# okieraised/rs-face-detection-tflite

Measured on AMD Instinct MI355X. Metric: faces/sec at batch=256 (256x256 back-camera) per GPU, higher is better.
Workload: dtype f32

## Files before the change

rs-face-detection-tflite_amd/csrc/engine.cpp:

```cpp
#include "engine.hpp"
#include "launch.hpp"

#include <algorithm>
#include <cstdio>
#include <cstdlib>
#include <cstring>
#include <stdexcept>

namespace mi {

void hip_check(hipError_t e, const char* what) {
    if (e != hipSuccess) throw std::runtime_error(std::string(what) + ": " + hipGetErrorString(e));
}

namespace {
template <class T>
void upload(T*& dev, std::vector<T>& host, const char* what_alloc, const char* what_copy) {
    if (dev) hip_check(hipFree(dev), "hipFree");
    dev = nullptr;
    if (host.empty()) return;
    hip_check(hipMalloc(reinterpret_cast<void**>(&dev), host.size() * sizeof(T)), what_alloc);
    hip_check(hipMemcpy(dev, host.data(), host.size() * sizeof(T), hipMemcpyHostToDevice), what_copy);
    std::vector<T>().swap(host);
}
// ... 53 lines not shown

const Model::Option* Model::find_option(const std::string& key) {
    using O = Option;
    constexpr int kMax = 0x7fffffff;
    static const Option table[] = {
        {"chunk", &Model::chunk_, 0, kMax, 0},
        {"graph", &Model::use_graph_, 0, 1, 0},
        {"fuse", &Model::fuse_level_, 0, 5, O::kReplan},
        {"res_budget", &Model::res_budget_, 16, 156, O::kReplan | O::kKiB},
        {"pipe", &Model::pipe_max_, 0, 4, O::kReplan},
        {"small_chain", &Model::small_chain_, 0, 64, O::kFreeSmall},
        {"pipe_rows", &Model::pipe_rows_, 1 << 1 | 1 << 2 | 1 << 4, 0, O::kOneOf},
        {"pipe_band", &Model::pipe_band_, 0, 4096, 0},
        {"strip", &Model::strip_, 0, 1, 0},
        {"stem_fuse", &Model::stem_fuse_, 0, 1, 0},
        {"stem_mfma", &Model::stem_mfma_, 0, 2, O::kForms},
        {"conv_mfma", &Model::conv_mfma_, 0, 1, 0},
        {"conv_bf16", &Model::conv_bf16_, 0, 2, O::kReplan},
        {"stem_run", &Model::stem_run_, 0, 32, 0},
        {"pair_fuse", &Model::pair_fuse_, 0, 1, 0},
        {"mdb_band", &Model::mdb_band_, 0, 4096, 0},
        {"chain_fixed", &Model::chain_fixed_, 0, 1, 0},
        {"chain_sched", &Model::chain_sched_, 0, 1, 0},
        {"mchain", &Model::mchain_, 0, 1, 0},
        {"tail", &Model::tail_, 0, 1, O::kReplan},
        {"tail_pre", &Model::tail_pre_, 0, 2, 0},
        {"tail_g", &Model::tail_g_, 0, 64, 0},
        {"band", &Model::band_, 0, 2, O::kReplan},
        {"band_test_fail", &Model::band_test_fail_, 0, 1, O::kWriteOnly},
        {"band_test_absent", &Model::band_test_absent_, 0, 256, O::kWriteOnly},
        {"band_test_gen", nullptr, 0, kMax, O::kBandGen | O::kWriteOnly},
        {"band_wide", &Model::band_wide_ok_, 0, 1, O::kReplan},
        {"band_fork", &Model::band_fork_, 0, 1, O::kReplan},
        {"band_nw", &Model::band_nw_, 8, 256, O::kReplan},
        {"band_fail_streak", &Model::band_fail_streak_, 0, 0, O::kReadOnly},
        {"band_wraps", &Model::band_wraps_, 0, 0, O::kReadOnly},
        {"fork", &Model::fork_, 0, 1, 0},
        {"heads", &Model::head_streams_opt_, 1, kHeadStreams, O::kReplan},
        {"reuse", &Model::reuse_, 0, 1, O::kReplan},
        {"lanes", &Model::lanes_, 1, 4, 0},
        {"test_poison", &Model::test_poison_, 1 << 1 | 1 << 2, 0, O::kOneOf | O::kKeepGraphs},
    };
    for (const Option& o : table)
        if (key == o.key) return &o;
    return nullptr;
}
// ... 198 lines not shown
}

LaunchCtx Model::launch_ctx(const float* in, int chunk_start, int frames) const {
    LaunchCtx c;
    c.weights = d_weights_;
    c.arena = d_arena_ + static_cast<size_t>(plan_.arena_floats_per_frame) * chunk_cap_ * arena_lane_;
    c.in = in; c.out = d_out_.data();
    c.small = d_small_; c.small_floats = small_floats_;
    c.progs = d_programs_; c.tail_progs = d_tail_programs_;
    c.band_prog = d_band_prog_; c.band_consts = d_band_consts_; c.band_ws = d_band_ws_; c.band_sync = d_band_sync_; c.band_fail = d_band_fail_;
    c.chunk_cap = chunk_cap_; c.chunk_start = chunk_start; c.F = frames;
    c.u8_frames = u8_.frames; c.u8_lut = u8_.lut; c.u8_frame_bytes = u8_.frame_bytes; c.u8_row_bytes = u8_.row_bytes;
    c.strip = strip_; c.pair_fuse = pair_fuse_; c.stem_fuse = stem_fuse_; c.stem_mfma = stem_mfma_; c.stem_run = stem_run_; c.mchain = mchain_; c.conv_mfma = conv_mfma_; c.conv_bf16 = conv_bf16_;
    c.small_chain = small_chain_; c.lanes = lanes_;
    c.pipe_rows = pipe_rows_; c.pipe_band = pipe_band_; c.mdb_band = mdb_band_; c.tail_pre = tail_pre_; c.tail_g = tail_g_;
    c.fork = fork_ && lanes_ == 1;
    c.cu_count = device_cu_count();
    c.band = band_use_ && chunk_start == 0;
    c.band_test_absent = band_test_absent_;
    return c;
}

namespace {
int issue(const Launch& l, hipStream_t s, int chain_fixed, int chain_sched) {
    auto many = [&](int (*f)(const BlockArgs*, int, void*)) { return f(l.blocks.data(), static_cast<int>(l.blocks.size()), s); };
    switch (l.to) {
        case Launcher::Conv: return launch_conv(std::get<ConvArgs>(l.args), s);
        case Launcher::HeadGemm: return launch_head_gemm(std::get<HeadGemmArgs>(l.args), s);
        case Launcher::Dw: return launch_dw(std::get<DwArgs>(l.args), s);
        case Launcher::Xc: return launch_xc(std::get<XcArgs>(l.args), s);
        case Launcher::Mdblock: return launch_mdblock(std::get<DblockArgs>(l.args), s);
        case Launcher::Dblock: return launch_dblock(std::get<DblockArgs>(l.args), s);
        case Launcher::Mbneck: return launch_mbneck(std::get<BneckArgs>(l.args), s);
        case Launcher::Bneck: return launch_bneck(std::get<BneckArgs>(l.args), s);
        case Launcher::Tail: return launch_tail(std::get<TailLaunch>(l.args), s);
        case Launcher::Resident: return launch_resident(std::get<ResLaunch>(l.args), s);
        case Launcher::Chain: return launch_chain(std::get<ChainArgs>(l.args), s, chain_fixed, chain_sched);
        case Launcher::StripPipe: return many(launch_strip_pipe);
        case Launcher::MstripChain: return many(launch_mstrip_chain);
        case Launcher::SmallChain: {
            int rc = 0;
            for (size_t k = 0; k < l.blocks.size() && rc == 0; k++) rc = l.blocks[k].sh == 1 ? launch_strip(l.blocks[k], s) : launch_block(l.blocks[k], s);
            return rc;
        }
        case Launcher::Ms2: return launch_ms2(std::get<BlockArgs>(l.args), s);
        case Launcher::Mwalk: return launch_mwalk(std::get<BlockArgs>(l.args), s);
        case Launcher::Strip: return launch_strip(std::get<BlockArgs>(l.args), s);
        case Launcher::Mstrip: return launch_mstrip(std::get<BlockArgs>(l.args), s);
        case Launcher::Block: return launch_block(std::get<BlockArgs>(l.args), s);
        case Launcher::Add: return launch_add(std::get<EltArgs>(l.args), s);
        case Launcher::Act: return launch_act(std::get<EltArgs>(l.args), s);
        case Launcher::Maxpool: return launch_maxpool(std::get<EltArgs>(l.args), s);
        case Launcher::Padc: return launch_padc(std::get<EltArgs>(l.args), s);
        case Launcher::Resize2x: return launch_resize2x(std::get<EltArgs>(l.args), s);
        case Launcher::DepthToSpace: return launch_depth_to_space(std::get<EltArgs>(l.args), s);
        case Launcher::Bandnet: return launch_bandnet(std::get<BandLaunch>(l.args), s);
        case Launcher::Avgpool: return launch_avgpool(std::get<EltArgs>(l.args), s);
        case Launcher::L2norm: return launch_l2norm_rows(std::get<EltArgs>(l.args), s);
        case Launcher::Transpose: return launch_transpose(std::get<EltArgs>(l.args), s);
    }
    return 0;
}
}

void Model::enqueue_chunk(const float* in, int chunk_start, int F, hipStream_t trunk, std::vector<hipEvent_t>* marks, Lowered* keep) {
    LaunchCtx ctx = launch_ctx(in, chunk_start, F);
    if (marks) ctx.fork = false;
    Lowered low = lower_chunk(plan_, consts_, band_plan_, sched_, ctx, keep != nullptr);
    auto mark = [&] {
        if (!marks) return;
        hipEvent_t ev;
// ... 8 lines not shown
        if (!head_events_[k]) hip_check(hipEventCreateWithFlags(&head_events_[k], hipEventDisableTiming), "hipEventCreate");
        return head_events_[k];
    };
    unsigned used_heads = 0;
    for (size_t k = 0; k < n_launches; k++) {
        const Launch& l = low.launches[k];
        hipStream_t s = trunk;
        if (l.slot >= 0) {
            while (static_cast<int>(head_streams_.size()) <= l.slot) {
                hipStream_t st;
                hip_check(hipStreamCreateWithFlags(&st, hipStreamNonBlocking), "hipStreamCreate");
                head_streams_.push_back(st);
            }
            s = head_streams_[static_cast<size_t>(l.slot)];
            if (l.wait >= 0) {
                hip_check(wait_event(s, event(static_cast<size_t>(low.launch_of_node[static_cast<size_t>(l.wait)]))), "hipStreamWaitEvent");
            } else {
                hip_check(record_event(event(start_event), trunk), "hipEventRecord");
                hip_check(wait_event(s, event(start_event)), "hipStreamWaitEvent");
            }
            used_heads |= 1u << l.slot;
        }
        int rc = 0;
        for (int rep = 0; rep < (marks ? profile_inner_ : 1) && rc == 0; rep++) rc = issue(l, s, chain_fixed_, chain_sched_);
        if (rc != 0) throw std::runtime_error(std::string("kernel launch failed: ") + hipGetErrorString(static_cast<hipError_t>(rc)));
        if (l.record) hip_check(record_event(event(k), s), "hipEventRecord");
        mark();
    }
    for (int k = 0; k < kHeadStreams; k++)
        if (used_heads & (1u << k)) {
            hip_check(record_event(event(start_event + 1 + static_cast<size_t>(k)), head_streams_[static_cast<size_t>(k)]), "hipEventRecord");
            hip_check(wait_event(trunk, event(start_event + 1 + static_cast<size_t>(k))), "hipStreamWaitEvent");
        }
    last_chunk_frames_ = F;
    if (keep) *keep = std::move(low);
}

void Model::enqueue_all(const float* in, int batch, hipStream_t s) {
    if (lanes_ > 1 && batch > chunk_cap_) {
        while (static_cast<int>(side_streams_.size()) < lanes_ - 1) {
            hipStream_t st;
            hip_check(hipStreamCreateWithFlags(&st, hipStreamNonBlocking), "hipStreamCreate");
            side_streams_.push_back(st);
        }
        while (static_cast<int>(lane_events_.size()) < lanes_) {
            hipEvent_t ev;
            hip_check(hipEventCreateWithFlags(&ev, hipEventDisableTiming), "hipEventCreate");
// ... 197 lines not shown
```

rs-face-detection-tflite_amd/csrc/engine.hpp:

```cpp
#pragma once

#include <hip/hip_runtime.h>

#include <map>
#include <memory>
#include <string>
#include <vector>

#include "bandplan.hpp"
#include "consts.hpp"
#include "launches.hpp"
#include "plan.hpp"

namespace mi {

void hip_check(hipError_t e, const char* what);

class Model {
   public:
    Model(const uint8_t* bytes, size_t n, int device);
    ~Model();
    Model(const Model&) = delete;
    Model& operator=(const Model&) = delete;

// ... 29 lines not shown
    void rebuild();
    struct Option;
    static const Option* find_option(const std::string& key);
    void build_bandnet();
    void free_bandnet();
    bool band_usable(int batch) const;
    void band_before_launch(hipStream_t s);
    void poison_scratch(hipStream_t s);
    void ensure_capacity(int batch);
    LaunchCtx launch_ctx(const float* in, int chunk_start, int frames) const;
    void enqueue_chunk(const float* in, int chunk_start, int frames, hipStream_t s, std::vector<hipEvent_t>* marks = nullptr, Lowered* keep = nullptr);
    void enqueue_all(const float* in, int batch, hipStream_t s);
    void invalidate_graphs();

    int device_ = 0;
    std::vector<uint8_t> blob_;
    Plan plan_;
    int fuse_level_ = 5, pipe_max_ = 4, tail_ = 1, reuse_ = 1;
    int res_budget_ = 156 * 1024;
    int chunk_ = 0, lanes_ = 1, use_graph_ = 1;
    int fork_ = 1, head_streams_opt_ = 1;
    int conv_mfma_ = 1;
    int conv_bf16_ = 0;
    int strip_ = 1, stem_fuse_ = 1, stem_mfma_ = 1, stem_run_ = 0, pair_fuse_ = 1, mchain_ = 1, chain_fixed_ = 1, chain_sched_ = 1;
    int pipe_rows_ = 0, pipe_band_ = 0, mdb_band_ = 0;
    int tail_pre_ = 0, tail_g_ = 0;
    int arena_lane_ = 0;
    std::vector<hipStream_t> side_streams_;
    std::vector<hipEvent_t> lane_events_;
    SideSchedule sched_;
    std::vector<hipStream_t> head_streams_;
    std::vector<hipEvent_t> head_events_;
    bool dirty_ = true;

    float* d_weights_ = nullptr;
    PlanConsts consts_;
    int profile_inner_ = 1;

    ResStage* d_programs_ = nullptr;
    TailStage* d_tail_programs_ = nullptr;
    float* d_arena_ = nullptr;
    size_t arena_floats_ = 0;
    int chunk_cap_ = 0;
    int batch_cap_ = 0;
    std::vector<float*> d_out_;
    float* d_in_stage_ = nullptr;
    size_t in_stage_floats_ = 0;
// ... 54 lines not shown
```

rs-face-detection-tflite_amd/csrc/kernels.hpp:

```cpp
#pragma once

#include <cstddef>
#include <cstdint>

namespace mi {

enum ActKind : int { ACT_NONE = 0, ACT_RELU = 1, ACT_RELU6 = 2, ACT_PRELU = 3 };
enum ResMode : int { RES_NONE = 0, RES_DIRECT = 1, RES_MAXPOOL = 2, RES_UP2X = 3 };

struct Epilogue {
    const float* bias = nullptr;
    const float* alpha = nullptr;
    const float* res = nullptr;
    long res_fs = 0;
    int res_mode = RES_NONE;
    int res_C = 0;
    int res_W = 0, res_H = 0;
    int act = ACT_NONE;
    int res_after = 0;
};

struct ConvArgs {
    const float* in = nullptr;
    const uint8_t* in_u8 = nullptr;
// ... 246 lines not shown
int launch_conv_bf16(const ConvArgs& a, void* stream);
int launch_dw(const DwArgs& a, void* stream);
int launch_block(const BlockArgs& a, void* stream);
bool block_kernel_supports(const BlockArgs& a);
const char* block_kernel_label(const BlockArgs& a, char* buf, size_t cap);
int launch_strip(const BlockArgs& a, void* stream);
bool strip_kernel_supports(const BlockArgs& a);
bool strip_shape_ok(int C, int Co);
int strip_consts_floats(int C);
void strip_pack_consts(int C, const float* w_dw, const float* b_dw, const float* w_pw, const float* bias, const float* alpha, int act, float* dst);
const char* strip_kernel_label(const BlockArgs& a, char* buf, size_t cap);
int launch_mwalk(const BlockArgs& a, void* stream);
bool mwalk_kernel_supports(const BlockArgs& a);
bool mwalk_shape_ok(int W, int C, int Co);
int mwalk_consts_floats(int W, int C, int Co);
void mwalk_pack_consts(int W, int C, int Co, const float* w_dw, const float* b_dw, const float* w_pw, const float* bias, const float* alpha, int act, float* dst);
const char* mwalk_kernel_label(const BlockArgs& a, char* buf, size_t cap);
int launch_ms2(const BlockArgs& a, void* stream);
bool ms2_kernel_supports(const BlockArgs& a);
bool ms2_shape_ok(int W, int C, int Co, bool skip);
int ms2_consts_floats(int W, int C, int Co, bool skip);
void ms2_pack_consts(int W, int C, int Co, bool skip, const float* w_dw, const float* b_dw, const float* w_pw, const float* bias, const float* alpha, int act, float* dst);
const char* ms2_kernel_label(const BlockArgs& a, char* buf, size_t cap);
int launch_mstrip(const BlockArgs& a, void* stream);
bool mstrip_kernel_supports(const BlockArgs& a);
bool mstrip_shape_ok(int C, int Co);
int mstrip_consts_floats(int C);
void mstrip_pack_consts(int C, const float* w_dw, const float* b_dw, const float* w_pw, const float* bias, const float* alpha, int act, float* dst);
const char* mstrip_kernel_label(const BlockArgs& a, char* buf, size_t cap);
bool mstrip_chain_supports(const BlockArgs* blocks, int n);
int launch_mstrip_chain(const BlockArgs* blocks, int n, void* stream);
bool strip_pipe_supports(const BlockArgs* blocks, int n);
bool strip_pipe_shape_ok(int C, int W);
bool strip_tail_shape_ok(int C, int Co, int H, int W);
int strip_consts_s2_floats(int C, int Co);
void strip_pack_consts_s2(int C, int Co, const float* w_dw, const float* b_dw, const float* w_pw, const float* bias, const float* alpha, int act, float* dst);
int launch_strip_pipe(const BlockArgs* blocks, int n, void* stream);
const char* strip_pipe_label(const BlockArgs* blocks, int n, char* buf, size_t cap);
int strip_pipe_rows_per_step(int H, int hint = 0);
int launch_chain(const ChainArgs& a, void* stream, int fixed = 1, int sched = 1);

struct BneckBlock {
    const float* w1 = nullptr;
    const float* w2 = nullptr;
    const float* consts = nullptr;
    float hi1 = 0.f, hi2 = 0.f;
    const float* mconsts = nullptr;
    int act1 = ACT_RELU, act2 = ACT_RELU;
};
constexpr int kMaxBneck = 6;
struct BneckArgs {
    const float* in = nullptr;
    float* out = nullptr;
    long in_fs = 0, out_fs = 0;
// ... 163 lines not shown
```

rs-face-detection-tflite_amd/csrc/mrow.hpp:

```cpp
#pragma once

#include <hip/hip_runtime.h>

#include <type_traits>
#include <utility>

#include "kernels.hpp"
#include "launch.hpp"
#include "wave_sync.hpp"

namespace mi {

namespace {

typedef float df32x4 __attribute__((ext_vector_type(4)));

__device__ __forceinline__ void dwg_barrier() {
    asm volatile("s_waitcnt lgkmcnt(0)\n\ts_barrier" ::: "memory");
}

template <class F, int... KS>
__device__ __forceinline__ void dfor_each(F&& f, std::integer_sequence<int, KS...>) { (f(std::integral_constant<int, KS>{}), ...); }

typedef float dv2f __attribute__((ext_vector_type(2)));
// ... 1 lines not shown
template <int WT>
struct RowAcc {
    dv2f p[WT / 2 ? WT / 2 : 1];
    float s[1];
    __device__ __forceinline__ void clear() {
#pragma unroll
        for (int q = 0; q < (WT / 2 ? WT / 2 : 1); q++) p[q] = dv2f{0.f, 0.f};
        s[0] = 0.f;
    }
};

template <int S>
__device__ __forceinline__ void dpk_fma(dv2f& acc, const dv2f x, const dv2f w) {
    if constexpr (S == 0) asm volatile("v_pk_fma_f32 %0, %1, %2, %0 op_sel:[0,0,0] op_sel_hi:[1,0,1]" : "+v"(acc) : "v"(x), "v"(w));
    else asm volatile("v_pk_fma_f32 %0, %1, %2, %0 op_sel:[0,1,0] op_sel_hi:[1,1,1]" : "+v"(acc) : "v"(x), "v"(w));
}
template <int S>
__device__ __forceinline__ dv2f dpk_mul(const dv2f x, const dv2f w) {
    dv2f r;
    if constexpr (S == 0) asm volatile("v_pk_mul_f32 %0, %1, %2 op_sel:[0,0] op_sel_hi:[1,0]" : "=v"(r) : "v"(x), "v"(w));
    else asm volatile("v_pk_mul_f32 %0, %1, %2 op_sel:[0,1] op_sel_hi:[1,1]" : "=v"(r) : "v"(x), "v"(w));
    return r;
}

__device__ __forceinline__ void dtaps_from(const float4 t0, const float4 t1, const float4 t2, dv2f (&t)[5]) {
    t[0] = dv2f{t0.x, t0.y}; t[1] = dv2f{t0.z, t0.w}; t[2] = dv2f{t1.x, t1.y}; t[3] = dv2f{t1.z, t1.w}; t[4] = dv2f{t2.x, 0.f};
}
template <int CK>
__device__ __forceinline__ void dload_taps(const float4* tp, dv2f (&tap)[CK][5]) {
#pragma unroll
    for (int ks = 0; ks < CK; ks++) dtaps_from(tp[ks * 12], tp[ks * 12 + 1], tp[ks * 12 + 2], tap[ks]);
#pragma unroll
    for (int ks = 0; ks < CK; ks++)
#pragma unroll
        for (int t = 0; t < 5; t++) asm volatile("" : "+v"(tap[ks][t]));
}

template <int CK, int MT, int WT, int PSV, bool EMIT, bool TAPL = false>
__device__ __forceinline__ void mdb_row(const unsigned src, const unsigned aop, const dv2f (&tap)[TAPL ? 1 : CK][5], RowAcc<WT> (&aPN)[CK], RowAcc<WT> (&aC)[CK],
                                        df32x4 (&D)[MT][WT], const float4* tapl = nullptr) {
    constexpr int NP = WT / 2, ODD = WT & 1;
    float xs[2][3][WT], av[2][MT];
    auto load_ks = [&](auto ksc, float (&x)[3][WT], float (&aw)[MT]) {
        constexpr int ks = decltype(ksc)::value;
        const unsigned xa = src, aa = aop;
#pragma unroll
// ... 89 lines not shown
        if constexpr (EMIT) {
#pragma unroll
            for (int mt = 0; mt < MT; mt++) asm volatile("ds_read_b32 %0, %1 offset:%2" : "=v"(aw[mt]) : "v"(aa), "n"((ks * MT + mt) * 64 * 4));
        }
    };
    auto landed = [&](float (&x)[3][2], float (&aw)[MT]) {
#pragma unroll
        for (int dx = 0; dx < 3; dx++) asm volatile("" : "+v"(x[dx][0]), "+v"(x[dx][1]));
        if constexpr (EMIT) {
#pragma unroll
            for (int mt = 0; mt < MT; mt++) asm volatile("" : "+v"(aw[mt]));
        }
    };
    auto kstep = [&](auto ksc) {
        constexpr int ks = decltype(ksc)::value;
        if constexpr (ks + 1 < CK) load_ks(std::integral_constant<int, ks + 1>{}, xs[(ks + 1) & 1], av[(ks + 1) & 1]);
        float (&x)[3][2] = xs[ks & 1];
        float (&aw)[MT] = av[ks & 1];
        const float (&w)[9] = tap[ks];
        float pch[2];
#pragma unroll
        for (int nt = 0; nt < 2; nt++) {
            float n = x[0][nt] * w[0], c = aC[ks][nt], pc = aPN[ks][nt];
#pragma unroll
            for (int dx = 0; dx < 3; dx++) {
                if (EMIT) pc = __builtin_fmaf(x[dx][nt], w[6 + dx], pc);
                if (dx) n = __builtin_fmaf(x[dx][nt], w[dx], n);
                c = __builtin_fmaf(x[dx][nt], w[3 + dx], c);
            }
            aC[ks][nt] = c;
            aPN[ks][nt] = n;
            asm volatile("" : "+v"(aC[ks][nt]), "+v"(aPN[ks][nt]));
            pch[nt] = pc;
        }
        if constexpr (EMIT) {
#pragma unroll
            for (int mt = 0; mt < MT; mt++) {
                D[mt][0] = __builtin_amdgcn_mfma_f32_16x16x4f32(aw[mt], pch[0], D[mt][0], 0, 0, 0);
                D[mt][1] = __builtin_amdgcn_mfma_f32_16x16x4f32(aw[mt], pch[1], D[mt][1], 0, 0, 0);
            }
        }
        asm volatile("s_waitcnt lgkmcnt(0)" ::: "memory");
        if constexpr (ks + 1 < CK) landed(xs[(ks + 1) & 1], av[(ks + 1) & 1]);
        __builtin_amdgcn_sched_barrier(0);
    };
    load_ks(std::integral_constant<int, 0>{}, xs[0], av[0]);
    asm volatile("s_waitcnt lgkmcnt(0)" ::: "memory");
    landed(xs[0], av[0]);
    __builtin_amdgcn_sched_barrier(0);
    dfor_each(kstep, std::make_integer_sequence<int, CK>{});
}


typedef __attribute__((address_space(1))) char gchar;
typedef __attribute__((address_space(1))) df32x4 gf32x4;

template <int CK>
__device__ __forceinline__ int mrow_goff(int lane) { return ((lane / (CK + 1)) * 4 * CK + 4 * min(lane % (CK + 1), CK - 1)) * 4; }

constexpr unsigned mrow_exec_hi(int active) { return active == 64 ? 0xffffffffu : (1u << (active - 32)) - 1; }

template <int C, int PS, int DPX, int ACTIVE>
// ... 124 lines not shown

template <int NST, int NLD>
__device__ __forceinline__ void mrow_wait(const bool st, const bool dm) {
    if (st && dm) wait_vm<NST + NLD>();
    else if (dm) wait_vm<NLD>();
    else if (st) wait_vm<NST>();
    else wait_vm<0>();
}

__device__ __forceinline__ void mrow_taps9(const float4* tp, float (&w)[9]) {
    const float4 t0 = tp[0], t1 = tp[1], t2 = tp[2];
    w[0] = t0.x; w[1] = t0.y; w[2] = t0.z; w[3] = t0.w; w[4] = t1.x; w[5] = t1.y; w[6] = t1.z; w[7] = t1.w; w[8] = t2.x;
}
template <int CK>
__device__ __forceinline__ void mrow_load_taps9(const float4* tp, float (&tap)[CK][9]) {
#pragma unroll
    for (int ks = 0; ks < CK; ks++) mrow_taps9(tp + ks * 12, tap[ks]);
#pragma unroll
    for (int ks = 0; ks < CK; ks++)
#pragma unroll
        for (int t = 0; t < 9; t++) asm volatile("" : "+v"(tap[ks][t]));
}


inline void mrow_pack_a(float* dst, const float* w_pw, int CK, int MT, int Co) {
    for (int ks = 0; ks < CK; ks++)
        for (int mt = 0; mt < MT; mt++)
            for (int l = 0; l < 64; l++) {
                const int o = 16 * mt + (l & 15);
                if (o < Co) dst[(ks * MT + mt) * 64 + l] = w_pw[(size_t)o * 4 * CK + 4 * ks + (l >> 4)];
            }
}
inline void mrow_pack_taps(float* dst, const float* w_dw, int CK) {
    for (int ks = 0; ks < CK; ks++)
        for (int kq = 0; kq < 4; kq++)
            for (int t = 0; t < 9; t++) dst[(ks * 4 + kq) * 12 + t] = w_dw[t * 4 * CK + 4 * ks + kq];
}
inline void mrow_pack_bias(float* dst_bias, float* dst_slope, int Co, int C, const float* w_pw, const float* b_dw, const float* bias, const float* alpha, int act) {
    for (int c = 0; c < Co; c++) {
        double acc = bias ? bias[c] : 0.0;
        if (b_dw)
            for (int k = 0; k < C; k++) acc += (double)w_pw[(size_t)c * C + k] * b_dw[k];
        dst_bias[c] = (float)acc;
        dst_slope[c] = act == ACT_PRELU ? alpha[c] : (act == ACT_NONE ? 1.f : 0.f);
    }
}
// ... 10 lines not shown
```

rs-face-detection-tflite_amd/csrc/mstrip_kernels.hip:

```cpp
#include <hip/hip_runtime.h>

#include <algorithm>
#include <cstdint>
#include <cstdio>
#include <cstdlib>
#include <type_traits>
#include <utility>

#include "kernels.hpp"
#include "launch.hpp"
#include "mrow.hpp"

namespace mi {

namespace {

struct MstripArgs {
    const float* in;
    float* out;
    const float* consts;
    long in_fs, out_fs;
    int B, H;
    int bands, band_rows;
    int has_res;
// ... 22 lines not shown
    static constexpr int NLD = 32 / DPX;
    static_assert(32 % DPX == 0 && NLD == 8, "eight DMA instructions per row (two source bases, four immediate offsets each)");
    static_assert((16 * PS) % 64 == 0 && 16 * PS / 64 < 256, "ds_read2st64_b32 reaches the second pixel tile");
    static constexpr int OFF_A = 0, A_F = CK * MT * 64, OFF_TAP = A_F, TAP_F = CK * 48, OFF_BIAS = OFF_TAP + TAP_F, OFF_SLOPE = OFF_BIAS + C, TOTAL = OFF_SLOPE + C;
    static constexpr int WG_F = A_F + 2 * C + TAP_F;
    static constexpr int NBUF = 2;
};

#ifdef MI_MSTRIP_STAMPS
struct MstripStamps { unsigned long long acc[7] = {0, 0, 0, 0, 0, 0, 0}, prev = __builtin_amdgcn_s_memtime(); };
#define MI_MSTAMP(k) { __builtin_amdgcn_sched_barrier(0); unsigned long long t_ = __builtin_amdgcn_s_memtime(); asm volatile("s_waitcnt lgkmcnt(0)" ::: "memory"); st.acc[k] += t_ - st.prev; st.prev = t_; __builtin_amdgcn_sched_barrier(0); }
#else
struct MstripStamps {};
#define MI_MSTAMP(k)
#endif

template <int CK>
__device__ __forceinline__ void mstrip_issue_row(const float* in, const int r, const int H, const unsigned lds_img, const int bi, const int goff) {
    using K = MK<CK>;
    mrow_dma2<K::C, K::PS, K::DPX, K::DPX * K::QP>(reinterpret_cast<const char*>(in + (long)min(max(r, 0), H - 1) * 32 * K::C),
                                                   lds_img + (unsigned)((bi * K::IMG_F + K::PS) * 4), goff);
}

template <int CK, bool RELU, class HR>
__device__ __forceinline__ void mstrip_walk(const float* in, float* out, const float* wgc, float* img, const unsigned lds_img, const int goff, const HR has_res,
                                            const float hi, const int H, const int y0, const int y1, const int lane, MstripStamps& st) {
    using K = MK<CK>;
    constexpr int C = K::C, MT = K::MT, PS = K::PS, QP = K::QP, IMG_F = K::IMG_F, NLD = K::NLD;
    const int kq = lane >> 4, p = lane & 15;
    float tap[CK][9];
    mrow_load_taps9<CK>(reinterpret_cast<const float4*>(wgc + K::A_F + 2 * C) + kq * 3, tap);
    MI_MSTAMP(0)
    typedef __attribute__((address_space(3))) float lfloat;
    const unsigned x_lds = (unsigned)(uintptr_t)(lfloat*)(img + p * PS + kq);
    const unsigned a_lds = (unsigned)(uintptr_t)(lfloat*)const_cast<float*>(wgc + lane);
    const float* sme = img + (1 + p) * PS + 4 * kq;
    const unsigned ooff = (unsigned)(p * C + 4 * kq) * 4u;

    float accA[CK][2], accB[CK][2];
    df32x4 D[MT][2];
#pragma unroll
    for (int ks = 0; ks < CK; ks++) accA[ks][0] = accA[ks][1] = accB[ks][0] = accB[ks][1] = 0.f;

    constexpr int NST = 2 * MT;
    auto step = [&](auto emit, int r, float (&aPN)[CK][2], float (&aC)[CK][2]) {
        const int t = r - (y0 - 1), bi = t & 1;
        mrow_wait<NST, NLD>(t - 1 >= 2, t == 0 || (t - 1) + 2 <= (y1 - y0 + 1));
        if (r < 0 || r >= H) mrow_clear_row<32 * QP>(img + bi * IMG_F + PS, lane);
        wave_sync();
        MI_MSTAMP(1)
        mstrip_row<CK, MT, PS, decltype(emit)::value>(x_lds + (unsigned)(bi * IMG_F * 4), a_lds, tap, aPN, aC, D);
        MI_MSTAMP(2)
        __builtin_amdgcn_sched_barrier(0);
        if constexpr (decltype(emit)::value) mrow_store_row<RELU, C, 32>(D, (gchar*)(out + (long)(r - 1) * 32 * C), ooff, wgc + K::A_F + C + 4 * kq, hi, p);
        MI_MSTAMP(3)
        __builtin_amdgcn_sched_barrier(0);
        mrow_init_acc<C, PS>(D, wgc + K::A_F + 4 * kq, sme + bi * IMG_F, has_res != 0);
        __builtin_amdgcn_sched_barrier(0);
        wave_sync();
        __builtin_amdgcn_s_waitcnt(0xC07F);
        if (r + 2 <= y1) mstrip_issue_row<CK>(in, r + 2, H, lds_img, bi, goff);
        MI_MSTAMP(4)
    };
    step(std::false_type{}, y0 - 1, accA, accB);
    step(std::false_type{}, y0, accB, accA);
    for (int r = y0 + 1; r <= y1; r += 2) {
        step(std::true_type{}, r, accA, accB);
        if (r + 1 > y1) break;
        step(std::true_type{}, r + 1, accB, accA);
    }
}

template <int CK, bool RELU>
__global__ __launch_bounds__(256, 2) void mstrip_kernel(MstripArgs a) {
    using K = MK<CK>;
    constexpr int C = K::C, PS = K::PS, QP = K::QP, IMG_F = K::IMG_F, NLD = K::NLD, NBUF = K::NBUF;
    extern __shared__ __attribute__((aligned(16))) float lds[];
    MstripStamps st;
    const int lane = threadIdx.x & 63;
    const int wave = __builtin_amdgcn_readfirstlane(threadIdx.x >> 6);
    float* wgc = lds;
    float* img = lds + K::WG_F + wave * NBUF * IMG_F;
    const int unit = blockIdx.x * 4 + wave;
    const int band = unit / a.B, b = unit - band * a.B;
    const bool active = band < a.bands;
    const int y0 = band * a.band_rows, y1 = min(y0 + a.band_rows, a.H);
    const float* in = a.in + (long)b * a.in_fs;
    const int goff = mrow_goff<CK>(lane);
    const unsigned lds_img = __builtin_amdgcn_readfirstlane((unsigned)(uintptr_t)(__attribute__((address_space(3))) float*)img);
    mrow_clear_border<QP, NBUF, IMG_F, 33 * PS>(img, lane);

    if (active) mstrip_issue_row<CK>(in, y0 - 1, a.H, lds_img, 0, goff);
    MI_MSTAMP(5)
    for (int i = threadIdx.x; i < K::A_F / 4; i += 256) reinterpret_cast<float4*>(wgc)[i] = reinterpret_cast<const float4*>(a.consts + K::OFF_A)[i];
    for (int i = threadIdx.x; i < 2 * C; i += 256) wgc[K::A_F + i] = a.consts[K::OFF_BIAS + i];
    for (int i = threadIdx.x; i < K::TAP_F / 4; i += 256) reinterpret_cast<float4*>(wgc + K::A_F + 2 * C)[i] = reinterpret_cast<const float4*>(a.consts + K::OFF_TAP)[i];
    if (active) mstrip_issue_row<CK>(in, y0, a.H, lds_img, 1, goff);
    if (active) wait_vm<NLD>(); else wait_vm<0>();
    MI_MSTAMP(6)
    asm volatile("s_waitcnt lgkmcnt(0)" ::: "memory");
    __builtin_amdgcn_s_barrier();
    asm volatile("" ::: "memory");
    if (!active) return;
    mstrip_walk<CK, RELU>(in, a.out + (long)b * a.out_fs, wgc, img, lds_img, goff, a.has_res != 0, a.hi, a.H, y0, y1, lane, st);
#ifdef MI_MSTRIP_STAMPS
    if (a.stamps && lane == 0)
        for (int k = 0; k < 7; k++) a.stamps[(long)unit * 8 + k] = st.acc[k];
#endif
}

template <int CK, bool RELU>
__global__ __launch_bounds__(512, 2) void mstrip_chain_kernel(MstripChainArgs ca) {
    using K = MK<CK>;
    constexpr int C = K::C, PS = K::PS, QP = K::QP, IMG_F = K::IMG_F, NLD = K::NLD, NBUF = K::NBUF;
    extern __shared__ __attribute__((aligned(16))) float lds[];
    MstripStamps st;
    const int lane = threadIdx.x & 63;
    const int wave = __builtin_amdgcn_readfirstlane(threadIdx.x >> 6);
    float* img = lds + 2 * K::WG_F + wave * NBUF * IMG_F;
    const int b = blockIdx.x;
    const int y0 = 4 * wave, y1 = y0 + 4;
    const int goff = mrow_goff<CK>(lane);
    const unsigned lds_img = __builtin_amdgcn_readfirstlane((unsigned)(uintptr_t)(__attribute__((address_space(3))) float*)img);
    mrow_clear_border<QP, NBUF, IMG_F, 33 * PS>(img, lane);

    for (int i = threadIdx.x; i < K::A_F / 4; i += 512) reinterpret_cast<float4*>(lds)[i] = reinterpret_cast<const float4*>(ca.consts[0] + K::OFF_A)[i];
    for (int i = threadIdx.x; i < 2 * C; i += 512) lds[K::A_F + i] = ca.consts[0][K::OFF_BIAS + i];
    for (int i = threadIdx.x; i < K::TAP_F / 4; i += 512) reinterpret_cast<float4*>(lds + K::A_F + 2 * C)[i] = reinterpret_cast<const float4*>(ca.consts[0] + K::OFF_TAP)[i];
    for (int blk = 0; blk < ca.nblocks; blk++) {
        float* wgc = lds + (blk & 1) * K::WG_F;
        const float* in = ca.in[blk] + (long)b * ca.in_fs[blk];
        const int has_res = ca.has_res[blk];
        const float hi = ca.hi[blk];
        float* const outp = ca.out[blk] + (long)b * ca.out_fs[blk];
        mstrip_issue_row<CK>(in, y0 - 1, ca.H, lds_img, 0, goff);
        constexpr int NPRE = (K::WG_F / 4 + 511) / 512;
        float4 pre[NPRE];
        const bool more = blk + 1 < ca.nblocks;
        if (more) {
            const float* cn = ca.consts[blk + 1];
#pragma unroll
            for (int k = 0; k < NPRE; k++) {
                const int i = threadIdx.x + 512 * k;
                const int src = i < K::A_F / 4 ? K::OFF_A + 4 * i : (i < (K::A_F + 2 * C) / 4 ? K::OFF_BIAS + 4 * i - K::A_F : K::OFF_TAP + 4 * i - K::A_F - 2 * C);
                pre[k] = i < K::WG_F / 4 ? *reinterpret_cast<const float4*>(cn + src) : make_float4(0.f, 0.f, 0.f, 0.f);
            }
        }
        mstrip_issue_row<CK>(in, y0, ca.H, lds_img, 1, goff);
        wait_vm<NLD>();
        asm volatile("s_waitcnt lgkmcnt(0)" ::: "memory");
        if (blk == 0) {
            __builtin_amdgcn_s_barrier();
            asm volatile("" ::: "memory");
        }
        mstrip_walk<CK, RELU>(in, outp, wgc, img, lds_img, goff, has_res, hi, ca.H, y0, y1, lane, st);
        asm volatile("s_waitcnt vmcnt(0)" ::: "memory");
        if (more) {
            float* nx = lds + ((blk + 1) & 1) * K::WG_F;
#pragma unroll
            for (int k = 0; k < NPRE; k++) {
                const int i = threadIdx.x + 512 * k;
                if (i < K::WG_F / 4) reinterpret_cast<float4*>(nx)[i] = pre[k];
            }
        }
        asm volatile("s_waitcnt vmcnt(0) lgkmcnt(0)" ::: "memory");
        __builtin_amdgcn_s_barrier();
        asm volatile("" ::: "memory");
    }
}

}

bool mstrip_shape_ok(int C, int Co) {
    static const bool off = getenv("MI_NO_MSTRIP") != nullptr;
    return !off && C == Co && C == 48;
}

bool mstrip_kernel_supports(const BlockArgs& a) {
// ... 14 lines not shown
    using K = MK<12>;
    std::fill(dst, dst + mstrip_consts_floats(C), 0.f);
    mrow_pack_a(dst + K::OFF_A, w_pw, C / 4, K::MT, C);
    mrow_pack_taps(dst + K::OFF_TAP, w_dw, C / 4);
    mrow_pack_bias(dst + K::OFF_BIAS, dst + K::OFF_SLOPE, C, C, w_pw, b_dw, bias, alpha, act);
}

const char* mstrip_kernel_label(const BlockArgs& a, char* buf, size_t cap) {
    snprintf(buf, cap, "mstrip_kernel<%d,%d>", a.C / 4, a.ep.act == ACT_RELU ? 1 : 0);
    return buf;
}

bool mstrip_chain_supports(const BlockArgs* blocks, int n) {
    static const bool off = getenv("MI_NO_MSTRIP_CHAIN") != nullptr;
    if (off || n < 2 || n > kMstripChain) return false;
    for (int k = 0; k < n; k++) {
        const BlockArgs& a = blocks[k];
        if (!mstrip_kernel_supports(a) || a.H != 32 || a.B != blocks[0].B || (a.ep.act == ACT_RELU) != (blocks[0].ep.act == ACT_RELU)) return false;
        if (k && a.in != blocks[k - 1].out) return false;
    }
    return true;
}

int launch_mstrip_chain(const BlockArgs* blocks, int n, void* stream) {
    using K = MK<12>;
    if (!mstrip_chain_supports(blocks, n)) return (int)hipErrorInvalidValue;
    MstripChainArgs ca{};
    ca.nblocks = n; ca.B = blocks[0].B; ca.H = blocks[0].H;
    for (int k = 0; k < n; k++) {
        const BlockArgs& a = blocks[k];
        ca.in[k] = a.in; ca.out[k] = a.out; ca.consts[k] = a.w_strip; ca.in_fs[k] = a.in_fs; ca.out_fs[k] = a.out_fs;
        ca.has_res[k] = a.ep.res_mode == RES_DIRECT;
        ca.hi[k] = a.ep.act == ACT_RELU6 ? 6.f : INFINITY;
    }
    const size_t lds_bytes = (size_t)(2 * K::WG_F + 8 * K::NBUF * K::IMG_F) * 4;
    return mrow_launch(mstrip_chain_kernel<12, true>, mstrip_chain_kernel<12, false>, blocks[0].ep.act == ACT_RELU, dim3((unsigned)ca.B), dim3(512), lds_bytes,
                       (hipStream_t)stream, ca);
}

unsigned long long* g_mstrip_stamps = nullptr;

int launch_mstrip(const BlockArgs& a, void* stream) {
    using K = MK<12>;
    MstripArgs ma;
    ma.stamps = g_mstrip_stamps;
    ma.in = a.in; ma.out = a.out; ma.consts = a.w_strip; ma.in_fs = a.in_fs; ma.out_fs = a.out_fs;
    ma.B = a.B; ma.H = a.H;
    static const int forced = getenv("MI_MSTRIP_BAND") ? atoi(getenv("MI_MSTRIP_BAND")) : 0;
    long bands = std::max<long>(1, (8L * device_cu_count() + a.B / 2) / std::max(1, a.B));
    int rows = (int)((a.H + bands - 1) / bands);
    rows = std::max(rows, std::min(a.H, 4));
    if (forced > 0) rows = std::min(forced, a.H);
    ma.band_rows = rows;
    ma.bands = (a.H + rows - 1) / rows;
    ma.has_res = a.ep.res_mode == RES_DIRECT;
    ma.hi = a.ep.act == ACT_RELU6 ? 6.f : INFINITY;
    const long units = (long)a.B * ma.bands;
    const size_t lds_bytes = (size_t)(K::WG_F + 4 * K::NBUF * K::IMG_F) * 4;
    return mrow_launch(mstrip_kernel<12, true>, mstrip_kernel<12, false>, a.ep.act == ACT_RELU, dim3((unsigned)((units + 3) / 4)), dim3(256), lds_bytes,
                       (hipStream_t)stream, ma);
}

}
```

Before: 223,600.

## Add packed-FMA depthwise row path with three-buffer accumulator rotation in mstrip

Adds a scheduled variant of the mstrip depthwise+pointwise row walk. Depthwise taps are packed into float pairs, and the 3x3 accumulation uses inline v_pk_fma_f32 on two output columns at once. The two-buffer accumulator swap becomes a three-buffer rotation (previous, current, next), with compile-time flags that skip dead depthwise work on the warm-up rows and the final row. The chain kernel gets a fixed row count of four so the walk can be fully specialised. The new path is on by default behind an mstrip_sched option. It raises register pressure and adds hand-written asm.

```diff
diff --git a/rs-face-detection-tflite_amd/csrc/engine.cpp b/rs-face-detection-tflite_amd/csrc/engine.cpp
--- a/rs-face-detection-tflite_amd/csrc/engine.cpp
+++ b/rs-face-detection-tflite_amd/csrc/engine.cpp
@@ -99,6 +99,7 @@
         {"mdb_band", &Model::mdb_band_, 0, 4096, 0},
         {"chain_fixed", &Model::chain_fixed_, 0, 1, 0},
         {"chain_sched", &Model::chain_sched_, 0, 1, 0},
+        {"mstrip_sched", &Model::mstrip_sched_, 0, 1, 0},
         {"mchain", &Model::mchain_, 0, 1, 0},
         {"tail", &Model::tail_, 0, 1, O::kReplan},
         {"tail_pre", &Model::tail_pre_, 0, 2, 0},
@@ -343,7 +344,7 @@
 }
 
 namespace {
-int issue(const Launch& l, hipStream_t s, int chain_fixed, int chain_sched) {
+int issue(const Launch& l, hipStream_t s, int chain_fixed, int chain_sched, int mstrip_sched) {
     auto many = [&](int (*f)(const BlockArgs*, int, void*)) { return f(l.blocks.data(), static_cast<int>(l.blocks.size()), s); };
     switch (l.to) {
         case Launcher::Conv: return launch_conv(std::get<ConvArgs>(l.args), s);
@@ -358,7 +359,7 @@
         case Launcher::Resident: return launch_resident(std::get<ResLaunch>(l.args), s);
         case Launcher::Chain: return launch_chain(std::get<ChainArgs>(l.args), s, chain_fixed, chain_sched);
         case Launcher::StripPipe: return many(launch_strip_pipe);
-        case Launcher::MstripChain: return many(launch_mstrip_chain);
+        case Launcher::MstripChain: return launch_mstrip_chain(l.blocks.data(), static_cast<int>(l.blocks.size()), s, mstrip_sched);
         case Launcher::SmallChain: {
             int rc = 0;
             for (size_t k = 0; k < l.blocks.size() && rc == 0; k++) rc = l.blocks[k].sh == 1 ? launch_strip(l.blocks[k], s) : launch_block(l.blocks[k], s);
@@ -367,7 +368,7 @@
         case Launcher::Ms2: return launch_ms2(std::get<BlockArgs>(l.args), s);
         case Launcher::Mwalk: return launch_mwalk(std::get<BlockArgs>(l.args), s);
         case Launcher::Strip: return launch_strip(std::get<BlockArgs>(l.args), s);
-        case Launcher::Mstrip: return launch_mstrip(std::get<BlockArgs>(l.args), s);
+        case Launcher::Mstrip: return launch_mstrip(std::get<BlockArgs>(l.args), s, mstrip_sched);
         case Launcher::Block: return launch_block(std::get<BlockArgs>(l.args), s);
         case Launcher::Add: return launch_add(std::get<EltArgs>(l.args), s);
         case Launcher::Act: return launch_act(std::get<EltArgs>(l.args), s);
@@ -422,7 +423,7 @@
             used_heads |= 1u << l.slot;
         }
         int rc = 0;
-        for (int rep = 0; rep < (marks ? profile_inner_ : 1) && rc == 0; rep++) rc = issue(l, s, chain_fixed_, chain_sched_);
+        for (int rep = 0; rep < (marks ? profile_inner_ : 1) && rc == 0; rep++) rc = issue(l, s, chain_fixed_, chain_sched_, mstrip_sched_);
         if (rc != 0) throw std::runtime_error(std::string("kernel launch failed: ") + hipGetErrorString(static_cast<hipError_t>(rc)));
         if (l.record) hip_check(record_event(event(k), s), "hipEventRecord");
         mark();
diff --git a/rs-face-detection-tflite_amd/csrc/engine.hpp b/rs-face-detection-tflite_amd/csrc/engine.hpp
--- a/rs-face-detection-tflite_amd/csrc/engine.hpp
+++ b/rs-face-detection-tflite_amd/csrc/engine.hpp
@@ -75,7 +75,7 @@
     int fork_ = 1, head_streams_opt_ = 1;
     int conv_mfma_ = 1;
     int conv_bf16_ = 0;
-    int strip_ = 1, stem_fuse_ = 1, stem_mfma_ = 1, stem_run_ = 0, pair_fuse_ = 1, mchain_ = 1, chain_fixed_ = 1, chain_sched_ = 1;
+    int strip_ = 1, stem_fuse_ = 1, stem_mfma_ = 1, stem_run_ = 0, pair_fuse_ = 1, mchain_ = 1, chain_fixed_ = 1, chain_sched_ = 1, mstrip_sched_ = 1;
     int pipe_rows_ = 0, pipe_band_ = 0, mdb_band_ = 0;
     int tail_pre_ = 0, tail_g_ = 0;
     int arena_lane_ = 0;
diff --git a/rs-face-detection-tflite_amd/csrc/kernels.hpp b/rs-face-detection-tflite_amd/csrc/kernels.hpp
--- a/rs-face-detection-tflite_amd/csrc/kernels.hpp
+++ b/rs-face-detection-tflite_amd/csrc/kernels.hpp
@@ -292,14 +292,14 @@
 int ms2_consts_floats(int W, int C, int Co, bool skip);
 void ms2_pack_consts(int W, int C, int Co, bool skip, const float* w_dw, const float* b_dw, const float* w_pw, const float* bias, const float* alpha, int act, float* dst);
 const char* ms2_kernel_label(const BlockArgs& a, char* buf, size_t cap);
-int launch_mstrip(const BlockArgs& a, void* stream);
+int launch_mstrip(const BlockArgs& a, void* stream, int sched = 1);
 bool mstrip_kernel_supports(const BlockArgs& a);
 bool mstrip_shape_ok(int C, int Co);
 int mstrip_consts_floats(int C);
 void mstrip_pack_consts(int C, const float* w_dw, const float* b_dw, const float* w_pw, const float* bias, const float* alpha, int act, float* dst);
 const char* mstrip_kernel_label(const BlockArgs& a, char* buf, size_t cap);
 bool mstrip_chain_supports(const BlockArgs* blocks, int n);
-int launch_mstrip_chain(const BlockArgs* blocks, int n, void* stream);
+int launch_mstrip_chain(const BlockArgs* blocks, int n, void* stream, int sched = 1);
 bool strip_pipe_supports(const BlockArgs* blocks, int n);
 bool strip_pipe_shape_ok(int C, int W);
 bool strip_tail_shape_ok(int C, int Co, int H, int W);
diff --git a/rs-face-detection-tflite_amd/csrc/mrow.hpp b/rs-face-detection-tflite_amd/csrc/mrow.hpp
--- a/rs-face-detection-tflite_amd/csrc/mrow.hpp
+++ b/rs-face-detection-tflite_amd/csrc/mrow.hpp
@@ -47,6 +47,25 @@
     else asm volatile("v_pk_mul_f32 %0, %1, %2 op_sel:[0,1] op_sel_hi:[1,1]" : "=v"(r) : "v"(x), "v"(w));
     return r;
 }
+
+#define MI_DPK_FMA(x, w, s) "v_pk_fma_f32 %0, " x ", " w ", %0 op_sel:[0," s ",0] op_sel_hi:[1," s ",1]"
+template <int S0, int S1, int S2>
+__device__ __forceinline__ void dpk_fma3(dv2f& acc, const dv2f x0, const dv2f x1, const dv2f x2, const dv2f w0, const dv2f w1, const dv2f w2) {
+    asm volatile(MI_DPK_FMA("%1", "%4", "%7") "\n\t" MI_DPK_FMA("%2", "%5", "%8") "\n\t" MI_DPK_FMA("%3", "%6", "%9")
+                 : "+v"(acc) : "v"(x0), "v"(x1), "v"(x2), "v"(w0), "v"(w1), "v"(w2), "n"(S0), "n"(S1), "n"(S2));
+}
+template <int S0, int S1>
+__device__ __forceinline__ void dpk_fma2(dv2f& acc, const dv2f x0, const dv2f x1, const dv2f w0, const dv2f w1) {
+    asm volatile(MI_DPK_FMA("%1", "%3", "%5") "\n\t" MI_DPK_FMA("%2", "%4", "%6") : "+v"(acc) : "v"(x0), "v"(x1), "v"(w0), "v"(w1), "n"(S0), "n"(S1));
+}
+template <int S0, int S1, int S2>
+__device__ __forceinline__ dv2f dpk_mul_fma2(const dv2f x0, const dv2f x1, const dv2f x2, const dv2f w0, const dv2f w1, const dv2f w2) {
+    dv2f r;
+    asm volatile("v_pk_mul_f32 %0, %1, %4 op_sel:[0,%7] op_sel_hi:[1,%7]\n\t" MI_DPK_FMA("%2", "%5", "%8") "\n\t" MI_DPK_FMA("%3", "%6", "%9")
+                 : "=&v"(r) : "v"(x0), "v"(x1), "v"(x2), "v"(w0), "v"(w1), "v"(w2), "n"(S0), "n"(S1), "n"(S2));
+    return r;
+}
+#undef MI_DPK_FMA
 
 __device__ __forceinline__ void dtaps_from(const float4 t0, const float4 t1, const float4 t2, dv2f (&t)[5]) {
     t[0] = dv2f{t0.x, t0.y}; t[1] = dv2f{t0.z, t0.w}; t[2] = dv2f{t1.x, t1.y}; t[3] = dv2f{t1.z, t1.w}; t[4] = dv2f{t2.x, 0.f};
@@ -182,12 +201,16 @@
 #pragma unroll
         for (int nt = 0; nt < 2; nt++) {
             float n = x[0][nt] * w[0], c = aC[ks][nt], pc = aPN[ks][nt];
+#ifdef MI_ABL_MSTRIP_NODW
+            if (EMIT) pc = x[1][nt];
+#else
 #pragma unroll
             for (int dx = 0; dx < 3; dx++) {
                 if (EMIT) pc = __builtin_fmaf(x[dx][nt], w[6 + dx], pc);
                 if (dx) n = __builtin_fmaf(x[dx][nt], w[dx], n);
                 c = __builtin_fmaf(x[dx][nt], w[3 + dx], c);
             }
+#endif
             aC[ks][nt] = c;
             aPN[ks][nt] = n;
             asm volatile("" : "+v"(aC[ks][nt]), "+v"(aPN[ks][nt]));
@@ -198,6 +221,70 @@
             for (int mt = 0; mt < MT; mt++) {
                 D[mt][0] = __builtin_amdgcn_mfma_f32_16x16x4f32(aw[mt], pch[0], D[mt][0], 0, 0, 0);
                 D[mt][1] = __builtin_amdgcn_mfma_f32_16x16x4f32(aw[mt], pch[1], D[mt][1], 0, 0, 0);
+            }
+        }
+        asm volatile("s_waitcnt lgkmcnt(0)" ::: "memory");
+        if constexpr (ks + 1 < CK) landed(xs[(ks + 1) & 1], av[(ks + 1) & 1]);
+        __builtin_amdgcn_sched_barrier(0);
+    };
+    load_ks(std::integral_constant<int, 0>{}, xs[0], av[0]);
+    asm volatile("s_waitcnt lgkmcnt(0)" ::: "memory");
+    landed(xs[0], av[0]);
+    __builtin_amdgcn_sched_barrier(0);
+    dfor_each(kstep, std::make_integer_sequence<int, CK>{});
+}
+
+template <int CK, int MT, int PS, bool DN, bool DC, bool EMIT>
+__device__ __forceinline__ void mstrip_row_pk(const unsigned xr, const unsigned ar, const dv2f (&tap)[9 * CK / 2], const dv2f (&aP)[CK], dv2f (&aC)[CK], dv2f (&aN)[CK],
+                                              df32x4 (&D)[MT][2]) {
+    float xs[2][3][2], av[2][MT];
+    auto load_ks = [&](auto ksc, float (&x)[3][2], float (&aw)[MT]) {
+        constexpr int ks = decltype(ksc)::value;
+        const unsigned xa = xr, aa = ar;
+#pragma unroll
+        for (int dx = 0; dx < 3; dx++) {
+            asm volatile("ds_read_b32 %0, %1 offset:%2" : "=v"(x[dx][0]) : "v"(xa), "n"((dx * PS + 4 * ks) * 4));
+            asm volatile("ds_read_b32 %0, %1 offset:%2" : "=v"(x[dx][1]) : "v"(xa), "n"((dx * PS + 4 * ks + 16 * PS) * 4));
+        }
+        if constexpr (EMIT) {
+#pragma unroll
+            for (int mt = 0; mt < MT; mt++) asm volatile("ds_read_b32 %0, %1 offset:%2" : "=v"(aw[mt]) : "v"(aa), "n"((ks * MT + mt) * 64 * 4));
+        }
+    };
+    auto landed = [&](float (&x)[3][2], float (&aw)[MT]) {
+#pragma unroll
+        for (int dx = 0; dx < 3; dx++) asm volatile("" : "+v"(x[dx][0]), "+v"(x[dx][1]));
+        if constexpr (EMIT) {
+#pragma unroll
+            for (int mt = 0; mt < MT; mt++) asm volatile("" : "+v"(aw[mt]));
+        }
+    };
+    auto kstep = [&](auto ksc) {
+        constexpr int ks = decltype(ksc)::value;
+        if constexpr (ks + 1 < CK) load_ks(std::integral_constant<int, ks + 1>{}, xs[(ks + 1) & 1], av[(ks + 1) & 1]);
+        float (&x)[3][2] = xs[ks & 1];
+        float (&aw)[MT] = av[ks & 1];
+        const dv2f x0 = dv2f{x[0][0], x[0][1]}, x1 = dv2f{x[1][0], x[1][1]}, x2 = dv2f{x[2][0], x[2][1]};
+        constexpr int f = 9 * ks;
+        dv2f pc = dv2f{0.f, 0.f};
+        if constexpr (EMIT) {
+            pc = aP[ks];
+            if constexpr (DN || DC) {
+                dpk_fma3<(f + 6) & 1, (f + 7) & 1, (f + 8) & 1>(pc, x0, x1, x2, tap[(f + 6) >> 1], tap[(f + 7) >> 1], tap[(f + 8) >> 1]);
+            } else {
+                dpk_fma2<(f + 6) & 1, (f + 7) & 1>(pc, x0, x1, tap[(f + 6) >> 1], tap[(f + 7) >> 1]);
+                const float w8 = (f + 8) & 1 ? tap[(f + 8) >> 1].y : tap[(f + 8) >> 1].x;
+                pc = dv2f{__builtin_fmaf(x2.x, w8, pc.x), __builtin_fmaf(x2.y, w8, pc.y)};
+            }
+        }
+        if constexpr (DN) aN[ks] = dpk_mul_fma2<f & 1, (f + 1) & 1, (f + 2) & 1>(x0, x1, x2, tap[f >> 1], tap[(f + 1) >> 1], tap[(f + 2) >> 1]);
+        if constexpr (DC) dpk_fma3<(f + 3) & 1, (f + 4) & 1, (f + 5) & 1>(aC[ks], x0, x1, x2, tap[(f + 3) >> 1], tap[(f + 4) >> 1], tap[(f + 5) >> 1]);
+        if constexpr (EMIT) {
+            if constexpr (DN || DC) __builtin_amdgcn_sched_barrier(0);
+#pragma unroll
+            for (int mt = 0; mt < MT; mt++) {
+                D[mt][0] = __builtin_amdgcn_mfma_f32_16x16x4f32(aw[mt], pc.x, D[mt][0], 0, 0, 0);
+                D[mt][1] = __builtin_amdgcn_mfma_f32_16x16x4f32(aw[mt], pc.y, D[mt][1], 0, 0, 0);
             }
         }
         asm volatile("s_waitcnt lgkmcnt(0)" ::: "memory");
@@ -368,6 +455,22 @@
         for (int t = 0; t < 9; t++) asm volatile("" : "+v"(tap[ks][t]));
 }
 
+template <int CK>
+__device__ __forceinline__ void mrow_load_taps_pk(const float4* tp, dv2f (&tap)[9 * CK / 2]) {
+    static_assert(CK % 2 == 0, "two k-steps fill nine pairs");
+#pragma unroll
+    for (int k2 = 0; k2 < CK / 2; k2++) {
+        float a[9], b[9];
+        mrow_taps9(tp + 2 * k2 * 12, a);
+        mrow_taps9(tp + (2 * k2 + 1) * 12, b);
+        dv2f* t = tap + 9 * k2;
+        t[0] = dv2f{a[0], a[1]}; t[1] = dv2f{a[2], a[3]}; t[2] = dv2f{a[4], a[5]}; t[3] = dv2f{a[6], a[7]}; t[4] = dv2f{a[8], b[0]};
+        t[5] = dv2f{b[1], b[2]}; t[6] = dv2f{b[3], b[4]}; t[7] = dv2f{b[5], b[6]}; t[8] = dv2f{b[7], b[8]};
+    }
+#pragma unroll
+    for (int q = 0; q < 9 * CK / 2; q++) asm volatile("" : "+v"(tap[q]));
+}
+
 
 inline void mrow_pack_a(float* dst, const float* w_pw, int CK, int MT, int Co) {
     for (int ks = 0; ks < CK; ks++)
diff --git a/rs-face-detection-tflite_amd/csrc/mstrip_kernels.hip b/rs-face-detection-tflite_amd/csrc/mstrip_kernels.hip
--- a/rs-face-detection-tflite_amd/csrc/mstrip_kernels.hip
+++ b/rs-face-detection-tflite_amd/csrc/mstrip_kernels.hip
@@ -68,14 +68,16 @@
                                                    lds_img + (unsigned)((bi * K::IMG_F + K::PS) * 4), goff);
 }
 
-template <int CK, bool RELU, class HR>
+template <int CK, bool RELU, int SCHED, int ROWS, class HR>
 __device__ __forceinline__ void mstrip_walk(const float* in, float* out, const float* wgc, float* img, const unsigned lds_img, const int goff, const HR has_res,
                                             const float hi, const int H, const int y0, const int y1, const int lane, MstripStamps& st) {
     using K = MK<CK>;
     constexpr int C = K::C, MT = K::MT, PS = K::PS, QP = K::QP, IMG_F = K::IMG_F, NLD = K::NLD;
     const int kq = lane >> 4, p = lane & 15;
-    float tap[CK][9];
-    mrow_load_taps9<CK>(reinterpret_cast<const float4*>(wgc + K::A_F + 2 * C) + kq * 3, tap);
+    float tap[SCHED ? 1 : CK][9];
+    dv2f tpk[SCHED ? 9 * CK / 2 : 1];
+    if constexpr (SCHED) mrow_load_taps_pk<CK>(reinterpret_cast<const float4*>(wgc + K::A_F + 2 * C) + kq * 3, tpk);
+    else mrow_load_taps9<CK>(reinterpret_cast<const float4*>(wgc + K::A_F + 2 * C) + kq * 3, tap);
     MI_MSTAMP(0)
     typedef __attribute__((address_space(3))) float lfloat;
     const unsigned x_lds = (unsigned)(uintptr_t)(lfloat*)(img + p * PS + kq);
@@ -83,19 +85,16 @@
     const float* sme = img + (1 + p) * PS + 4 * kq;
     const unsigned ooff = (unsigned)(p * C + 4 * kq) * 4u;
 
-    float accA[CK][2], accB[CK][2];
     df32x4 D[MT][2];
-#pragma unroll
-    for (int ks = 0; ks < CK; ks++) accA[ks][0] = accA[ks][1] = accB[ks][0] = accB[ks][1] = 0.f;
 
     constexpr int NST = 2 * MT;
-    auto step = [&](auto emit, int r, float (&aPN)[CK][2], float (&aC)[CK][2]) {
+    auto step = [&](auto emit, int r, auto&& row) {
         const int t = r - (y0 - 1), bi = t & 1;
         mrow_wait<NST, NLD>(t - 1 >= 2, t == 0 || (t - 1) + 2 <= (y1 - y0 + 1));
         if (r < 0 || r >= H) mrow_clear_row<32 * QP>(img + bi * IMG_F + PS, lane);
         wave_sync();
         MI_MSTAMP(1)
-        mstrip_row<CK, MT, PS, decltype(emit)::value>(x_lds + (unsigned)(bi * IMG_F * 4), a_lds, tap, aPN, aC, D);
+        row(x_lds + (unsigned)(bi * IMG_F * 4));
         MI_MSTAMP(2)
         __builtin_amdgcn_sched_barrier(0);
         if constexpr (decltype(emit)::value) mrow_store_row<RELU, C, 32>(D, (gchar*)(out + (long)(r - 1) * 32 * C), ooff, wgc + K::A_F + C + 4 * kq, hi, p);
@@ -108,16 +107,54 @@
         if (r + 2 <= y1) mstrip_issue_row<CK>(in, r + 2, H, lds_img, bi, goff);
         MI_MSTAMP(4)
     };
-    step(std::false_type{}, y0 - 1, accA, accB);
-    step(std::false_type{}, y0, accB, accA);
-    for (int r = y0 + 1; r <= y1; r += 2) {
-        step(std::true_type{}, r, accA, accB);
-        if (r + 1 > y1) break;
-        step(std::true_type{}, r + 1, accB, accA);
-    }
-}
-
-template <int CK, bool RELU>
+    using T = std::true_type;
+    using F = std::false_type;
+    if constexpr (SCHED) {
+        dv2f R0[CK], R1[CK], R2[CK];
+        auto stp = [&](auto dn, auto dc, auto emit, int r, dv2f (&aP)[CK], dv2f (&aC)[CK], dv2f (&aN)[CK]) {
+            step(emit, r, [&](const unsigned xr) {
+                mstrip_row_pk<CK, MT, PS, decltype(dn)::value, decltype(dc)::value, decltype(emit)::value>(xr, a_lds, tpk, aP, aC, aN, D);
+            });
+        };
+        stp(T{}, F{}, F{}, y0 - 1, R2, R2, R0);
+        stp(T{}, T{}, F{}, y0, R2, R0, R1);
+        if constexpr (ROWS) {
+            for (int r = y0 + 1;; r += 3) {
+                if (r == y0 + ROWS) { stp(F{}, F{}, T{}, r, R0, R1, R2); break; }
+                stp(T{}, T{}, T{}, r, R0, R1, R2);
+                if (r + 1 == y0 + ROWS) { stp(F{}, F{}, T{}, r + 1, R1, R2, R0); break; }
+                stp(T{}, T{}, T{}, r + 1, R1, R2, R0);
+                if (r + 2 == y0 + ROWS) { stp(F{}, F{}, T{}, r + 2, R2, R0, R1); break; }
+                stp(T{}, T{}, T{}, r + 2, R2, R0, R1);
+            }
+        } else {
+            for (int r = y0 + 1;; r += 3) {
+                stp(T{}, T{}, T{}, r, R0, R1, R2);
+                if (r == y1) break;
+                stp(T{}, T{}, T{}, r + 1, R1, R2, R0);
+                if (r + 1 == y1) break;
+                stp(T{}, T{}, T{}, r + 2, R2, R0, R1);
+                if (r + 2 == y1) break;
+            }
+        }
+    } else {
+        float accA[CK][2], accB[CK][2];
+#pragma unroll
+        for (int ks = 0; ks < CK; ks++) accA[ks][0] = accA[ks][1] = accB[ks][0] = accB[ks][1] = 0.f;
+        auto stp = [&](auto emit, int r, float (&aPN)[CK][2], float (&aC)[CK][2]) {
+            step(emit, r, [&](const unsigned xr) { mstrip_row<CK, MT, PS, decltype(emit)::value>(xr, a_lds, tap, aPN, aC, D); });
+        };
+        stp(F{}, y0 - 1, accA, accB);
+        stp(F{}, y0, accB, accA);
+        for (int r = y0 + 1; r <= y1; r += 2) {
+            stp(T{}, r, accA, accB);
+            if (r + 1 > y1) break;
+            stp(T{}, r + 1, accB, accA);
+        }
+    }
+}
+
+template <int CK, bool RELU, int SCHED>
 __global__ __launch_bounds__(256, 2) void mstrip_kernel(MstripArgs a) {
     using K = MK<CK>;
     constexpr int C = K::C, PS = K::PS, QP = K::QP, IMG_F = K::IMG_F, NLD = K::NLD, NBUF = K::NBUF;
@@ -148,14 +185,14 @@
     __builtin_amdgcn_s_barrier();
     asm volatile("" ::: "memory");
     if (!active) return;
-    mstrip_walk<CK, RELU>(in, a.out + (long)b * a.out_fs, wgc, img, lds_img, goff, a.has_res != 0, a.hi, a.H, y0, y1, lane, st);
+    mstrip_walk<CK, RELU, SCHED, 0>(in, a.out + (long)b * a.out_fs, wgc, img, lds_img, goff, a.has_res != 0, a.hi, a.H, y0, y1, lane, st);
 #ifdef MI_MSTRIP_STAMPS
     if (a.stamps && lane == 0)
         for (int k = 0; k < 7; k++) a.stamps[(long)unit * 8 + k] = st.acc[k];
 #endif
 }
 
-template <int CK, bool RELU>
+template <int CK, bool RELU, int SCHED>
 __global__ __launch_bounds__(512, 2) void mstrip_chain_kernel(MstripChainArgs ca) {
     using K = MK<CK>;
     constexpr int C = K::C, PS = K::PS, QP = K::QP, IMG_F = K::IMG_F, NLD = K::NLD, NBUF = K::NBUF;
@@ -199,7 +236,7 @@
             __builtin_amdgcn_s_barrier();
             asm volatile("" ::: "memory");
         }
-        mstrip_walk<CK, RELU>(in, outp, wgc, img, lds_img, goff, has_res, hi, ca.H, y0, y1, lane, st);
+        mstrip_walk<CK, RELU, SCHED, 4>(in, outp, wgc, img, lds_img, goff, has_res, hi, ca.H, y0, y1, lane, st);
         asm volatile("s_waitcnt vmcnt(0)" ::: "memory");
         if (more) {
             float* nx = lds + ((blk + 1) & 1) * K::WG_F;
@@ -260,7 +297,7 @@
     return true;
 }
 
-int launch_mstrip_chain(const BlockArgs* blocks, int n, void* stream) {
+int launch_mstrip_chain(const BlockArgs* blocks, int n, void* stream, int sched) {
     using K = MK<12>;
     if (!mstrip_chain_supports(blocks, n)) return (int)hipErrorInvalidValue;
     MstripChainArgs ca{};
@@ -272,13 +309,15 @@
         ca.hi[k] = a.ep.act == ACT_RELU6 ? 6.f : INFINITY;
     }
     const size_t lds_bytes = (size_t)(2 * K::WG_F + 8 * K::NBUF * K::IMG_F) * 4;
-    return mrow_launch(mstrip_chain_kernel<12, true>, mstrip_chain_kernel<12, false>, blocks[0].ep.act == ACT_RELU, dim3((unsigned)ca.B), dim3(512), lds_bytes,
-                       (hipStream_t)stream, ca);
+    const bool relu = blocks[0].ep.act == ACT_RELU;
+    const dim3 grid((unsigned)ca.B), block(512);
+    if (sched) return mrow_launch(mstrip_chain_kernel<12, true, 1>, mstrip_chain_kernel<12, false, 1>, relu, grid, block, lds_bytes, (hipStream_t)stream, ca);
+    return mrow_launch(mstrip_chain_kernel<12, true, 0>, mstrip_chain_kernel<12, false, 0>, relu, grid, block, lds_bytes, (hipStream_t)stream, ca);
 }
 
 unsigned long long* g_mstrip_stamps = nullptr;
 
-int launch_mstrip(const BlockArgs& a, void* stream) {
+int launch_mstrip(const BlockArgs& a, void* stream, int sched) {
     using K = MK<12>;
     MstripArgs ma;
     ma.stamps = g_mstrip_stamps;
@@ -295,8 +334,10 @@
     ma.hi = a.ep.act == ACT_RELU6 ? 6.f : INFINITY;
     const long units = (long)a.B * ma.bands;
     const size_t lds_bytes = (size_t)(K::WG_F + 4 * K::NBUF * K::IMG_F) * 4;
-    return mrow_launch(mstrip_kernel<12, true>, mstrip_kernel<12, false>, a.ep.act == ACT_RELU, dim3((unsigned)((units + 3) / 4)), dim3(256), lds_bytes,
-                       (hipStream_t)stream, ma);
-}
-
-}
+    const bool relu = a.ep.act == ACT_RELU;
+    const dim3 grid((unsigned)((units + 3) / 4)), block(256);
+    if (sched) return mrow_launch(mstrip_kernel<12, true, 1>, mstrip_kernel<12, false, 1>, relu, grid, block, lds_bytes, (hipStream_t)stream, ma);
+    return mrow_launch(mstrip_kernel<12, true, 0>, mstrip_kernel<12, false, 0>, relu, grid, block, lds_bytes, (hipStream_t)stream, ma);
+}
+
+}
```

New measurement: 225,200 (median of 6 runs). No clear change (+0.7%).
